# c-sommer/gradient-sdf

Measured on AMD Instinct MI355X. Metric: depth frames/sec fused+tracked, 640x480 @1cm voxels, higher is better.
Workload: dtype f32; 1 GPU; S-tum: TUM fr1/xyz-format synthetic stream, 640x480, 1 cm voxels, trunc 10, capacity 2^22 (BASELINE.json configs[1]); width=640, height=480, hash_capacity_log2=22, tracker=25 iters, conv 1e-3, damping 1, next_depth_hint=True, parallelism=replicas x1 (tracked path does not shard), full=False, burn_in_windows=2, converged_frames=20, voxels=1169329, n_upd_per_frame=4508803, n_hit_per_pass=254696

## Files before the change

gradient-sdf_amd/csrc/gsdf_capi.hip:

```cpp
#include "../../include/gsdf.h"
#include "../../include/gsdf_mc_tables.h"
#include "gsdf_ctx.h"
#include "gsdf_kernels.h"
#include "gsdf_math.h"

#include <hip/hip_runtime.h>

#include <algorithm>
#include <chrono>
#include <cmath>
#include <cstdio>
#include <cstdlib>
#include <cstring>
#include <numeric>
#include <string>
#include <thread>
#include <vector>

static int fail(int code, const std::string& msg) { return gsdf_fail(code, msg); }

namespace {

hipEvent_t take_event(gsdf_ctx* c) {
    if (!c->event_pool.empty()) {
        hipEvent_t e = c->event_pool.back();
        c->event_pool.pop_back();
        return e;
    }
    hipEvent_t e = nullptr;
    (void)hipEventCreateWithFlags(&e, hipEventDisableSystemFence);
    return e;
}

struct prof_scope {
    gsdf_ctx* c; int which; hipEvent_t a = nullptr, b = nullptr;
    prof_scope(gsdf_ctx* c_, int w) : c(c_), which(w) {
        if (c->profiling) { a = take_event(c); b = take_event(c); (void)hipEventRecord(a, c->stream); }
    }
    ~prof_scope() {
        if (c->profiling) { (void)hipEventRecord(b, c->stream); c->prof_events[which].push_back({ a, b }); }
    }
};

void prof_collect(gsdf_ctx* c) {
    for (int k = 0; k < GSDF_PROF_SLOTS; ++k) {
        for (auto& pr : c->prof_events[k]) {
            float ms = 0.f;
            if (hipEventElapsedTime(&ms, pr.first, pr.second) == hipSuccess) {
                c->prof_ms[k] += ms; c->prof_n[k] += 1;
                if (c->prof_each[k].size() < (size_t)1 << 20) c->prof_each[k].push_back(ms);
            }
            c->event_pool.push_back(pr.first);
            c->event_pool.push_back(pr.second);
        }
        c->prof_events[k].clear();
    }
}

int status_to_code(int status) {
    if (status & GSDF_STATUS_TABLE_FULL) return fail(GSDF_ERR_TABLE_FULL, "voxel hash table full (probe budget exhausted)");
    if (status & GSDF_STATUS_KEY_RANGE) return fail(GSDF_ERR_KEY_RANGE, "voxel index outside the packable +-2^20 range");
    if (status & GSDF_STATUS_TRACK_ABORT)
        return fail(GSDF_ERR_HIP, "tracking: the workgroups of the one-launch optimize() were not co-resident (GPU shared with another "
                                  "process?); that optimize() was abandoned -- set GSDF_PERSIST=0 to use one launch per pass");
    return GSDF_OK;
}

int require_frame(gsdf_ctx* c) {
    if (!c) return fail(GSDF_ERR_INVALID, "null context");
    if (!c->frame.planes) return fail(GSDF_ERR_INVALID, "gsdf_normals_init must be called first (NEst == nullptr, MapGradPixelSdf.cpp:55-58)");
    return GSDF_OK;
}

static int fuse_far_table(const gsdf_ctx* c) {
#ifdef GSDF_EXPERIMENTS
    if (c->debug & 1024) return 1;
    if (c->debug & 2048) return 0;
#endif
    if (c->far_table >= 0) return c->far_table;
    return c->progress && c->progress[3] * 16u > (unsigned int)c->fuse_blocks ? 1 : 0;
}

static inline void cpu_relax() {
#if defined(__x86_64__) || defined(__i386__)
    __builtin_ia32_pause();
#else
    std::this_thread::yield();
// ... 323 lines not shown
}

}

int gsdf_flush_pending(gsdf_ctx* c) {
    if (!c || !c->ahead.pending.valid) return GSDF_OK;
    c->ahead.release();
    if (hipSetDevice(c->device) != hipSuccess) return fail(GSDF_ERR_HIP, "hipSetDevice");
    const size_t N = (size_t)c->W * c->H;
    const gsdf_lookahead::pending_fuse& p = c->ahead.pending;
    return launch_fuse(c, p.depth, c->frame.normals + (size_t)p.set * 3 * N, p.pose, 0, fuse_far_table(c), nullptr, nullptr);
}
#define GSDF_FLUSH(c) do { if ((c) && (c)->ahead.pending.valid) { const int rc_ = gsdf_flush_pending(c); if (rc_) return rc_; } } while (0)
static int flush_if_overlaps(gsdf_ctx* c, const void* dst, int64_t bytes) {
    if (c && c->ahead.range_changes(dst, (size_t)std::max<int64_t>(bytes, 0), c->frame_bytes())) return gsdf_flush_pending(c);
    return GSDF_OK;
}

extern "C" {

const char* gsdf_last_error(void) { return g_gsdf_err.c_str(); }
#ifdef GSDF_EXPERIMENTS
#define GSDF_TRACE_WG 8192
#define GSDF_TRACE_COLS 16
int gsdf_debug_flags(gsdf_ctx* c, int flags) {
    GSDF_FLUSH(c);
    if (!c) return GSDF_ERR_INVALID;
    c->debug = flags;
    if (flags & 64) {
        if (hipStreamSynchronize(c->stream) != hipSuccess) return GSDF_ERR_HIP;
        if (!c->trace && c->trace.alloc((size_t)GSDF_TRACE_WG * GSDF_TRACE_COLS) != hipSuccess) return GSDF_ERR_HIP;
        if (hipMemset(c->trace, 0, (size_t)GSDF_TRACE_WG * GSDF_TRACE_COLS * 8) != hipSuccess) return GSDF_ERR_HIP;
        const unsigned long long ptr = (unsigned long long)(uintptr_t)c->trace.get();
        if (hipMemcpy(&c->st->dbg[23], &ptr, 8, hipMemcpyHostToDevice) != hipSuccess) return GSDF_ERR_HIP;
    }
    return GSDF_OK;
}
int gsdf_debug_trace(gsdf_ctx* c, unsigned long long* out, int n_wg) {
    GSDF_FLUSH(c);
    if (!c || !out || !c->trace || n_wg > GSDF_TRACE_WG) return GSDF_ERR_INVALID;
    if (hipStreamSynchronize(c->stream) != hipSuccess) return GSDF_ERR_HIP;
    if (hipMemcpy(out, c->trace, (size_t)n_wg * GSDF_TRACE_COLS * 8, hipMemcpyDeviceToHost) != hipSuccess) return GSDF_ERR_HIP;
    return GSDF_OK;
}
int gsdf_debug_raycast_rows(gsdf_ctx* c, unsigned long long* out, int n_rows) {
    GSDF_FLUSH(c);
    if (!c || !out || !c->rc_counts || (size_t)n_rows > c->rc_counts.count() / 8) return GSDF_ERR_INVALID;
    if (hipStreamSynchronize(c->stream) != hipSuccess) return GSDF_ERR_HIP;
    if (hipMemcpy(out, c->rc_counts, (size_t)n_rows * 8 * sizeof(unsigned long long), hipMemcpyDeviceToHost) != hipSuccess) return GSDF_ERR_HIP;
    return GSDF_OK;
}
int gsdf_debug_tile_counters(gsdf_ctx* c, unsigned long long* out, int n_rows) {
    GSDF_FLUSH(c);
    if (!c || !out || !c->frame.blk_counters || n_rows > c->fuse_blocks) return GSDF_ERR_INVALID;
    if (hipStreamSynchronize(c->stream) != hipSuccess) return GSDF_ERR_HIP;
    if (hipMemcpy(out, c->frame.blk_counters, (size_t)n_rows * 4 * sizeof(unsigned long long), hipMemcpyDeviceToHost) != hipSuccess) return GSDF_ERR_HIP;
    return GSDF_OK;
}
int gsdf_debug_set_tile_order(gsdf_ctx* c, const uint32_t* order, int n) {
    GSDF_FLUSH(c);
    if (!c || !order || !c->frame.tile_order || n != c->fuse_blocks) return GSDF_ERR_INVALID;
    if (hipStreamSynchronize(c->stream) != hipSuccess) return GSDF_ERR_HIP;
    if (hipMemcpy(c->frame.tile_order, order, (size_t)n * sizeof(uint32_t), hipMemcpyHostToDevice) != hipSuccess) return GSDF_ERR_HIP;
    return GSDF_OK;
}
int gsdf_debug_get_tile_order(gsdf_ctx* c, uint32_t* order, int* n) {
    if (!c || !order || !n || !c->frame.tile_order) return GSDF_ERR_INVALID;
    if (hipMemcpy(order, c->frame.tile_order, (size_t)c->fuse_blocks * sizeof(uint32_t), hipMemcpyDeviceToHost) != hipSuccess) return GSDF_ERR_HIP;
    *n = c->fuse_blocks;
    return GSDF_OK;
}
int gsdf_debug_read(gsdf_ctx* c, unsigned long long out[24]) {
    GSDF_FLUSH(c);
    if (!c || !out) return GSDF_ERR_INVALID;
    if (hipStreamSynchronize(c->stream) != hipSuccess) return GSDF_ERR_HIP;
    gsdf_dev_state h;
    if (hipMemcpy(&h, c->st, sizeof(h), hipMemcpyDeviceToHost) != hipSuccess) return GSDF_ERR_HIP;
    for (int i = 0; i < 24; ++i) out[i] = h.dbg[i];
    return GSDF_OK;
}
int gsdf_debug_normals_tile_split(int tiles, int k, int launches, int iters, int batch, int nrm_split, int nrm_split2, int* lo, int* hi) {
    return lo && hi && normals_tile_split(tiles, k, launches, iters, batch, nrm_split, nrm_split2, lo, hi) ? 1 : 0;
}
int gsdf_debug_fail_alloc(int nth) {
    const int made = g_gsdf_alloc_count;
    g_gsdf_alloc_count = 0;
    g_gsdf_alloc_fail_at = nth > 0 ? nth : 0;
    return made;
}
const char* gsdf_version(void) { return "gsdf-mi355x 0.2 (gfx950) +experiments"; }
#else
const char* gsdf_version(void) { return "gsdf-mi355x 0.2 (gfx950)"; }
#endif

static int create_impl(gsdf_ctx** out, float voxel_size, float trunc_dist, int capacity_log2, int device, bool other_queue);
int gsdf_create(gsdf_ctx** out, float voxel_size, float trunc_dist, int capacity_log2, int device) {
    return create_impl(out, voxel_size, trunc_dist, capacity_log2, device, false);
}
int gsdf_create_shards(gsdf_ctx** out, int n, float voxel_size, float trunc_dist, int capacity_log2, int device) {
    if (!out || n < 1 || n > 4) return fail(GSDF_ERR_INVALID, "gsdf_create_shards: 1..4 contexts (one hardware queue each)");
    for (int i = 0; i < n; ++i) out[i] = nullptr;
    for (int i = 0; i < n; ++i) {
        const int rc = create_impl(&out[i], voxel_size, trunc_dist, capacity_log2, device, true);
        if (rc) { for (int j = 0; j < i; ++j) { gsdf_destroy(out[j]); out[j] = nullptr; } return rc; }
    }
    return GSDF_OK;
}
static int create_impl(gsdf_ctx** out, float voxel_size, float trunc_dist, int capacity_log2, int device, bool other_queue) {
    if (!out) return fail(GSDF_ERR_INVALID, "out == NULL");
    *out = nullptr;
    if (!(voxel_size > 0.f) || !(trunc_dist > 0.f)) return fail(GSDF_ERR_INVALID, "voxel_size and trunc_dist must be > 0");
    if (capacity_log2 < 10 || capacity_log2 > 30) return fail(GSDF_ERR_INVALID, "capacity_log2 must be in [10, 30]");
    if (!(trunc_dist < 2.f)) return fail(GSDF_ERR_INVALID, "trunc_dist must be < 2 m (fixed-point range of the fusion kernel's accumulators)");
    int n_dev = 0;
    if (hipGetDeviceCount(&n_dev) != hipSuccess || n_dev <= 0) {
        (void)hipGetLastError();
        return fail(GSDF_ERR_NO_DEVICE, "no HIP device visible: libgsdf has no CPU fallback");
    }
    if (device < 0 || device >= n_dev) return fail(GSDF_ERR_INVALID, "device ordinal out of range");
    HIP_TRY(hipSetDevice(device));
    gsdf_ctx* c = new gsdf_ctx();
    c->device = device;
    c->voxel_size = voxel_size;
    c->voxel_size_inv = (float)(1. / voxel_size);
    c->T = trunc_dist;
    c->inv_T = (float)(1. / trunc_dist);
    c->factor = (int)std::floor(c->T / c->voxel_size);
    c->capacity_log2 = capacity_log2;
    c->n_slots = (size_t)1 << capacity_log2;
    hipError_t e;
    int prio_least = 0, prio_greatest = 0;
    if (other_queue) {
        if (hipDeviceGetStreamPriorityRange(&prio_least, &prio_greatest) != hipSuccess || prio_greatest == prio_least) {
            (void)hipGetLastError();
            delete c;
            return fail(GSDF_ERR_HIP, "gsdf_create_shards: the device offers no stream priority range, so separate hardware queues cannot be guaranteed (use gsdf_create)");
        }
    }
    if ((e = (other_queue ? hipStreamCreateWithPriority(&c->stream, hipStreamNonBlocking, prio_greatest)
                          : hipStreamCreateWithFlags(&c->stream, hipStreamNonBlocking))) != hipSuccess ||
        (e = c->map.alloc(c->n_slots, 0)) != hipSuccess || (e = c->st.alloc(1)) != hipSuccess || (e = c->counter.alloc(1)) != hipSuccess ||
        (e = hipEventCreate(&c->ev0)) != hipSuccess || (e = hipEventCreate(&c->ev1)) != hipSuccess) {
        std::string m = std::string("gsdf_create: ") + hipGetErrorString(e);
        gsdf_destroy(c);
        return fail(GSDF_ERR_HIP, m);
    }
    {
        const char* env = getenv("GSDF_DEFER");
        if (env) c->defer = atoi(env);
    }
    c->tab = c->map.table(c->n_slots);
    {
        if (c->progress.alloc(16) != hipSuccess) (void)hipGetLastError();
        const char* env = getenv("GSDF_ADAPTIVE");
        if (env) c->adaptive = atoi(env);
        if ((env = getenv("GSDF_FIRST_BATCH")) && atoi(env) >= 2) c->first_batch = atoi(env);
        if ((env = getenv("GSDF_FUSE_HEAD"))) c->fuse_head = atoi(env) != 0;
        if ((env = getenv("GSDF_NRM_SPLIT"))) {
            int a = -1, b = -1;
            const int n = sscanf(env, "%d,%d", &a, &b);
            if (n >= 1 && a >= 0 && a <= 100) { c->nrm_split = a; c->nrm_split2 = 100 - a; }
            if (n >= 2 && b >= 0 && a + b <= 100) c->nrm_split2 = b;
        }
        if ((env = getenv("GSDF_NEXT_BATCH")) && atoi(env) >= 1) c->next_batch = atoi(env);
        if ((env = getenv("GSDF_LAZY_FUSE"))) c->lazy_fuse = atoi(env);
        if ((env = getenv("GSDF_PERSIST"))) c->persist = atoi(env);
// ... 1098 lines not shown
```

gradient-sdf_amd/csrc/gsdf_kernels.hip:

```cpp
#include "gsdf_kernels.h"

#ifdef GSDF_EXPERIMENTS
#define GSDF_EXPERIMENT(flags, mask) (((flags) & (mask)) != 0)
#define GSDF_TRACE(a, tr, col) do { if (GSDF_EXPERIMENT((a).debug, 64) && threadIdx.x == 0) (tr)[col] = wall_clock64(); } while (0)
#else
#define GSDF_EXPERIMENT(flags, mask) (false)
#define GSDF_TRACE(a, tr, col) do { } while (0)
#endif
#include "gsdf_math.h"

#include <hip/hip_runtime.h>
#include <algorithm>
#include <cstring>
#include <vector>

#define FULL_MASK 0xFFFFFFFFFFFFFFFFull

template <int CTRL, int ROW_MASK>
__device__ __forceinline__ float dpp_add(float v) {
    const int moved = __builtin_amdgcn_update_dpp(0, __float_as_int(v), CTRL, ROW_MASK, 0xf, false);
    return v + __int_as_float(moved);
}
__device__ __forceinline__ float wave_sum(float v) {
    v = dpp_add<0x111, 0xf>(v);
    v = dpp_add<0x112, 0xf>(v);
    v = dpp_add<0x114, 0xf>(v);
    v = dpp_add<0x118, 0xf>(v);
    v = dpp_add<0x142, 0xa>(v);
    v = dpp_add<0x143, 0xc>(v);
    return __int_as_float(__builtin_amdgcn_readlane(__float_as_int(v), 63));
}

template <int CTRL, int ROW_MASK>
__device__ __forceinline__ uint32_t dpp_umin(uint32_t v) {
    const uint32_t m = (uint32_t)__builtin_amdgcn_update_dpp((int)0xFFFFFFFFu, (int)v, CTRL, ROW_MASK, 0xf, false);
    return m < v ? m : v;
}
template <int CTRL, int ROW_MASK>
__device__ __forceinline__ uint32_t dpp_umax(uint32_t v) {
    const uint32_t m = (uint32_t)__builtin_amdgcn_update_dpp(0, (int)v, CTRL, ROW_MASK, 0xf, false);
    return m > v ? m : v;
}
__device__ __forceinline__ void wave_uminmax(uint32_t& lo, uint32_t& hi) {
    lo = dpp_umin<0x111, 0xf>(lo); hi = dpp_umax<0x111, 0xf>(hi);
    lo = dpp_umin<0x112, 0xf>(lo); hi = dpp_umax<0x112, 0xf>(hi);
    lo = dpp_umin<0x114, 0xf>(lo); hi = dpp_umax<0x114, 0xf>(hi);
    lo = dpp_umin<0x118, 0xf>(lo); hi = dpp_umax<0x118, 0xf>(hi);
    lo = dpp_umin<0x142, 0xa>(lo); hi = dpp_umax<0x142, 0xa>(hi);
    lo = dpp_umin<0x143, 0xc>(lo); hi = dpp_umax<0x143, 0xc>(hi);
    lo = (uint32_t)__builtin_amdgcn_readlane((int)lo, 63);
    hi = (uint32_t)__builtin_amdgcn_readlane((int)hi, 63);
}

#define GSDF_DPP_STAGE(CTRL)                                                                     \
    _Pragma("unroll") for (int i = 0; i < N; ++i)                                                \
        asm volatile("v_add_f32_dpp %0, %0, %0 " CTRL : "+v"(v[i]))
template <int N>
__device__ __forceinline__ void wave_sum_to_lane63(float (&v)[N]) {
    static_assert(N >= 3, "DPP read-after-write distance");
    if constexpr (N == 29) {
        asm volatile("s_nop 1" : "+v"(v[0]), "+v"(v[1]), "+v"(v[2]), "+v"(v[3]), "+v"(v[4]), "+v"(v[5]), "+v"(v[6]), "+v"(v[7]), "+v"(v[8]),
                     "+v"(v[9]), "+v"(v[10]), "+v"(v[11]), "+v"(v[12]), "+v"(v[13]), "+v"(v[14]), "+v"(v[15]), "+v"(v[16]), "+v"(v[17]), "+v"(v[18]),
                     "+v"(v[19]), "+v"(v[20]), "+v"(v[21]), "+v"(v[22]), "+v"(v[23]), "+v"(v[24]), "+v"(v[25]), "+v"(v[26]), "+v"(v[27]), "+v"(v[28]));
    } else {
#pragma unroll
        for (int i = 0; i < N; ++i) asm volatile("s_nop 1" : "+v"(v[i]));
    }
    GSDF_DPP_STAGE("row_shr:1 row_mask:0xf bank_mask:0xf bound_ctrl:1");
    GSDF_DPP_STAGE("row_shr:2 row_mask:0xf bank_mask:0xf bound_ctrl:1");
    GSDF_DPP_STAGE("row_shr:4 row_mask:0xf bank_mask:0xf bound_ctrl:1");
    GSDF_DPP_STAGE("row_shr:8 row_mask:0xf bank_mask:0xf bound_ctrl:1");
    GSDF_DPP_STAGE("row_bcast:15 row_mask:0xa bank_mask:0xf");
    GSDF_DPP_STAGE("row_bcast:31 row_mask:0xc bank_mask:0xf");
}
#undef GSDF_DPP_STAGE

__device__ __forceinline__ int reflect101(int i, int n) {
    if (n == 1) return 0;
    while (i < 0 || i >= n) {
        if (i < 0) i = -i;
        else i = 2 * (n - 1) - i;
    }
    return i;
}

__global__ __launch_bounds__(256) void k_table_clear(gsdf_table tab, size_t n_blocks) {
    const size_t stride = (size_t)gridDim.x * blockDim.x;
    const size_t n16 = n_blocks * GSDF_BLOCK_VOX * 2;
    uint4* p = reinterpret_cast<uint4*>(tab.vox);
    for (size_t i = (size_t)blockIdx.x * blockDim.x + threadIdx.x; i < n16; i += stride) p[i] = make_uint4(0u, 0u, 0u, 0u);
    for (size_t i = (size_t)blockIdx.x * blockDim.x + threadIdx.x; i < n_blocks; i += stride) tab.bkeys[i] = GSDF_KEY_EMPTY;
    const size_t n_occ = ((size_t)gsdf_occ_mask(tab) + 1) / 32 + ((size_t)gsdf_occ2_mask(tab) + 1) / 32;
// ... 1279 lines not shown
    float trig[4] = { 0.f, 1.f, 0.f, 1.f };
    const float theta_sq = gsdf_se3_theta_sq(xi);
    if (!(theta_sq < GSDF_SOPHUS_EPS * GSDF_SOPHUS_EPS)) {
        const float theta = sqrtf(theta_sq), half = 0.5f * theta;
        const float arg = (threadIdx.x & 1u) ? theta : half;
        const float sn = sinf(arg), cs = cosf(arg);
        trig[0] = trk_lane_value(sn, 0); trig[1] = trk_lane_value(cs, 0);
        trig[2] = trk_lane_value(sn, 1); trig[3] = trk_lane_value(cs, 1);
    }
    gsdf_se3_exp_mul_trig(xi, pose7, trig);
}
__device__ __forceinline__ float trk_sin_small(float x, float x2) {
    float p = __builtin_fmaf(x2, -1.f / 5040.f, 1.f / 120.f);
    p = __builtin_fmaf(x2, p, -1.f / 6.f);
    return __builtin_fmaf(x, x2 * p, x);
}
__device__ __forceinline__ float trk_cos_small(float x2) {
    float p = __builtin_fmaf(x2, -1.f / 720.f, 1.f / 24.f);
    p = __builtin_fmaf(x2, p, -0.5f);
    return __builtin_fmaf(x2, p, 1.f);
}
__device__ __forceinline__ void trk_se3_exp_mul_fast(const float* xi, float* pose7) {
    const float theta_sq = gsdf_se3_theta_sq(xi);
    if (__builtin_expect(!(theta_sq >= GSDF_SOPHUS_EPS * GSDF_SOPHUS_EPS && theta_sq < 0.01f), 0)) {
        trk_se3_exp_mul_wave(xi, pose7);
        return;
    }
    const float rth = trk_rsq(theta_sq);
    const float theta = theta_sq * rth, half = 0.5f * theta;
    const float tsq = theta * theta, hsq = half * half;
    const float rth2 = rth * rth;
    const float imag = trk_sin_small(half, hsq) * rth;
    const float real = trk_cos_small(hsq);
    const float a = (1.f - trk_cos_small(tsq)) * rth2;
    const float b = (theta - trk_sin_small(theta, tsq)) * (rth2 * rth);
    float qn[4];
    gsdf_se3_exp_mul_parts(xi, pose7, imag, real, false, a, b, qn);
    const float rl = trk_rsq(qn[0] * qn[0] + qn[1] * qn[1] + qn[2] * qn[2] + qn[3] * qn[3]);
#pragma unroll
    for (int i = 0; i < 4; ++i) pose7[3 + i] = qn[i] * rl;
}

__device__ __forceinline__ void trk_solve_update(const float* tot, float damping, float conv_sq, int passes, int max_passes,
                                                 int no_solve, bool exact_solve ,
                                                 float pose[7], int* done, int* converged) {
    float gvec[6], Hm[36];
#pragma unroll
    for (int i = 0; i < 6; ++i) gvec[i] = tot[1 + i];
    int q = 7;
#pragma unroll
    for (int i = 0; i < 6; ++i)
#pragma unroll
        for (int j = i; j < 6; ++j) { Hm[6 * i + j] = tot[q]; Hm[6 * j + i] = tot[q]; ++q; }
    float xi[6];
    if (no_solve) { for (int i = 0; i < 6; ++i) xi[i] = 1.f; }
    else if (exact_solve || __builtin_expect(!trk_llt_solve6_fast(Hm, gvec, xi), 0))
        gsdf_llt_solve6(Hm, gvec, xi);
#pragma unroll
    for (int i = 0; i < 6; ++i) xi[i] = damping * xi[i];
    const float nrm = gsdf_sum3(xi[0] * xi[0], xi[1] * xi[1], xi[2] * xi[2]) +
                      gsdf_sum3(xi[3] * xi[3], xi[4] * xi[4], xi[5] * xi[5]);
    *done = 0; *converged = 0;
    if (nrm < conv_sq) {
        *converged = 1;
        *done = 1;
    } else {
        bool nan = false;
#pragma unroll
        for (int i = 0; i < 6; ++i) nan = nan || isnan(xi[i]);
        if (!nan && !no_solve) {
            float mxi[6];
#pragma unroll
            for (int i = 0; i < 6; ++i) mxi[i] = -xi[i];
            if (exact_solve) trk_se3_exp_mul_wave(mxi, pose);
            else trk_se3_exp_mul_fast(mxi, pose);
        }
        if (passes >= max_passes) *done = 1;
    }
}

template <int PPT>
__device__ __forceinline__ void trk_gather(const gsdf_frame_geom& g, const gsdf_table& tab, const float* __restrict__ depth,
                                           const float* z_first, const float pose[7], int pix0, int pix_stride, int batch_stride,
                                           float (&acc)[GSDF_TRACK_NSUM], unsigned long long* wave_stamp = nullptr,
                                           const int xy_scale = 1) {
    const unsigned long long ws_t0 = wave_stamp ? wall_clock64() : 0ull;
    float R[9];
    gsdf_quat_to_R(pose + 3, R);
    const float t[3] = { pose[0], pose[1], pose[2] };
    const float fx_inv = 1.f / g.fx, fy_inv = 1.f / g.fy;
    const int N = g.W * g.H;
    const uint32_t uW = (uint32_t)g.W;
    const uint32_t step_y = (uint32_t)pix_stride / uW, step_x = (uint32_t)pix_stride - step_y * uW;
    for (int base = pix0; base < N; base += batch_stride) {
        float z[PPT];
        bool ok[PPT];
#pragma unroll
        for (int j = 0; j < PPT; ++j) {
            const int pix = base + j * pix_stride;
            ok[j] = pix < N;
            z[j] = (z_first && base == pix0) ? z_first[j] : (ok[j] ? depth[pix] : 0.f);
        }
        gsdf_v3 p[PPT];
        int vx[PPT], vy[PPT], vz[PPT];
        unsigned long long key[PPT], bkey[PPT], k0[PPT];
        uint32_t home[PPT];
        uint32_t px, py = (uint32_t)base / uW;
        px = (uint32_t)base - py * uW;
#pragma unroll
        for (int j = 0; j < PPT; ++j) {
            ok[j] = ok[j] && !(z[j] <= g.zmin || z[j] >= g.zmax);
            const int y = (int)py * xy_scale, x = (int)px * xy_scale;
            px += step_x; py += step_y;
            if (px >= uW) { px -= uW; ++py; }
            const float x0 = ((float)x - g.cx) * fx_inv;
            const float y0 = ((float)y - g.cy) * fy_inv;
            const gsdf_v3 pc = { x0 * z[j], y0 * z[j], z[j] };
            const gsdf_v3 Rp = gsdf_matvec(R, pc);
            p[j] = gsdf_v3{ Rp.x + t[0], Rp.y + t[1], Rp.z + t[2] };
            vx[j] = gsdf_float2vox1(g.inv_vs, p[j].x);
            vy[j] = gsdf_float2vox1(g.inv_vs, p[j].y);
            vz[j] = gsdf_float2vox1(g.inv_vs, p[j].z);
            ok[j] = ok[j] && gsdf_key_in_range(vx[j], vy[j], vz[j]);
            key[j] = gsdf_key_pack(vx[j], vy[j], vz[j]);
            bkey[j] = gsdf_block_key(key[j]);
            home[j] = gsdf_hash(bkey[j]) & tab.block_mask;
            k0[j] = ok[j] ? tab.bkeys[home[j]] : GSDF_KEY_EMPTY;
        }
        const gsdf_payload* P[PPT];
        float2 pa[PPT], pb[PPT], pc2[PPT];
        int blk[PPT];
        {
            uint32_t want = 0u;
#pragma unroll
            for (int j = 0; j < PPT; ++j) want |= ok[j] ? 1u << j : 0u;
            gsdf_block_lookup_n<PPT, false>(tab, bkey, home, k0, want, blk);
        }
        unsigned long long ws_lookup = 0ull, ws_ok = 0ull;
        if (wave_stamp && base == pix0) {
            ws_lookup = wall_clock64() - ws_t0;
#pragma unroll
            for (int j = 0; j < PPT; ++j) ws_ok += (unsigned long long)__popcll(__ballot(ok[j]));
        }
#pragma unroll
        for (int j = 0; j < PPT; ++j) {
            P[j] = blk[j] >= 0 ? tab.vox + ((size_t)blk[j] * GSDF_BLOCK_VOX + gsdf_block_local(key[j])) : nullptr;
            if (P[j]) {
                const float2* q = reinterpret_cast<const float2*>(P[j]);
                pa[j] = q[0]; pb[j] = q[1]; pc2[j] = q[2];
            } else {
                pa[j] = make_float2(0.f, 0.f); pb[j] = pa[j]; pc2[j] = pa[j];
            }
        }
#pragma unroll
        for (int j = 0; j < PPT; ++j) {
            const float w0 = pa[j].x;
            if (!(w0 > 0.f)) continue;
            const gsdf_v3 gn = gsdf_normalized3(gsdf_v3{ pb[j].x, pb[j].y, pc2[j].x });
            const gsdf_v3 gr = { 1.2f * gn.x, 1.2f * gn.y, 1.2f * gn.z };
            const gsdf_v3 d = { g.vs * (float)vx[j] - p[j].x, g.vs * (float)vy[j] - p[j].y, g.vs * (float)vz[j] - p[j].z };
            const float phi = gsdf_tsdf_phi(pa[j].y / w0, gn, d);
            const gsdf_v3 pxg = gsdf_cross3(p[j], gr);
            const float J[6] = { gr.x, gr.y, gr.z, pxg.x, pxg.y, pxg.z };
            acc[0] += phi * phi;
#pragma unroll
            for (int i = 0; i < 6; ++i) acc[1 + i] += phi * J[i];
            int q = 7;
#pragma unroll
            for (int i = 0; i < 6; ++i)
#pragma unroll
                for (int jj = i; jj < 6; ++jj) acc[q++] += J[i] * J[jj];
            acc[28] += 1.f;
        }
        if (wave_stamp && base == pix0) {
            unsigned long long hits = 0ull;
#pragma unroll
            for (int j = 0; j < PPT; ++j) hits += (unsigned long long)__popcll(__ballot(pa[j].x > 0.f));
            const unsigned long long tot = wall_clock64() - ws_t0;
            if ((threadIdx.x & 63) == 0)
                *wave_stamp = (tot & 0xFFFFull) | ((ws_lookup & 0xFFFFull) << 16) | ((ws_ok & 0xFFFFull) << 32) | ((hits & 0xFFFFull) << 48);
        }
    }
}

struct base_sample {
    float w;
    float phi;
    gsdf_v3 grad;
};
__device__ __forceinline__ base_sample gsdf_base_sample(const gsdf_table& tab, float inv_vs, float T, gsdf_v3 p) {
    const float pi = inv_vs * p.x, pj = inv_vs * p.y, pk = inv_vs * p.z;
    const int im = (int)floorf(pi), jm = (int)floorf(pj), km = (int)floorf(pk);
    const float dx = pi - (float)im, dy = pj - (float)jm, dz = pk - (float)km;
    const uint32_t inx = (gsdf_key_in_range(im, 0, 0) ? 1u : 0u) | (gsdf_key_in_range(im + 1, 0, 0) ? 2u : 0u);
    const uint32_t iny = (gsdf_key_in_range(0, jm, 0) ? 1u : 0u) | (gsdf_key_in_range(0, jm + 1, 0) ? 2u : 0u);
    const uint32_t inz = (gsdf_key_in_range(0, 0, km) ? 1u : 0u) | (gsdf_key_in_range(0, 0, km + 1) ? 2u : 0u);
    const uint32_t span = ((im & 3) == 3 ? 1u : 0u) | ((jm & 3) == 3 ? 2u : 0u) | ((km & 3) == 3 ? 4u : 0u);
    unsigned long long bk[8], k[8];
    uint32_t h[8];
    int blk[8];
    uint32_t pend = 0u;
#pragma unroll
    for (int e = 0; e < 8; ++e) {
        const int i0 = e & 1, j0 = (e >> 1) & 1, k0 = (e >> 2) & 1;
        const bool want = (e & ~span) == 0u && ((inx >> i0) & 1u) && ((iny >> j0) & 1u) && ((inz >> k0) & 1u);
        bk[e] = want ? gsdf_block_key(gsdf_key_pack(im + i0, jm + j0, km + k0)) : 0ull;
        h[e] = gsdf_hash(bk[e]) & tab.block_mask;
        k[e] = want ? tab.bkeys[h[e]] : GSDF_KEY_EMPTY;
        pend |= want ? 1u << e : 0u;
    }
    gsdf_block_lookup_n<8, false>(tab, bk, h, k, pend, blk);
    float d[8], wv[8];
    uint32_t present = 0u;
#pragma unroll
    for (int c = 0; c < 8; ++c) {
        int b = blk[0];
#pragma unroll
        for (int e = 1; e < 8; ++e)
            if ((e & ~c) == 0) b = (uint32_t)e == (c & span) ? blk[e] : b;
// ... 28 lines not shown
    const float d13 = (1.f - dy) * d[1] + dy * d[3];
    const float d46 = (1.f - dy) * d[4] + dy * d[6];
    const float d57 = (1.f - dy) * d[5] + dy * d[7];
    r.grad.x = inv_vs * ((1.f - dz) * d13 + dz * d57 - (1.f - dz) * d02 - dz * d46);
    r.grad.y = inv_vs * ((1.f - dz) * d23 + dz * d67 - (1.f - dz) * d01 - dz * d45);
    r.grad.z = inv_vs * ((1.f - dy) * d45 + dy * d67 - (1.f - dy) * d01 - dy * d23);
    const float dy0 = (1.f - dy) * d01 + dy * d23;
    const float dy1 = (1.f - dy) * d45 + dy * d67;
    r.phi = (1.f - dz) * dy0 + dz * dy1;
    return r;
}

template <int PPT>
__device__ __forceinline__ void trk_gather_base(const gsdf_frame_geom& g, const gsdf_table& tab, const float* __restrict__ depth,
                                                const float pose[7], int pix0, int pix_stride, int batch_stride,
                                                float (&acc)[GSDF_TRACK_NSUM], const int xy_scale = 1) {
    float R[9];
    gsdf_quat_to_R(pose + 3, R);
    const float t[3] = { pose[0], pose[1], pose[2] };
    const float fx_inv = 1.f / g.fx, fy_inv = 1.f / g.fy;
    const int N = g.W * g.H;
    const uint32_t uW = (uint32_t)g.W;
#pragma unroll 1
    for (int base = pix0; base < N; base += batch_stride) {
#pragma unroll 1
        for (int j = 0; j < PPT; ++j) {
            const int pix = base + j * pix_stride;
            if (pix >= N) break;
            const float z = depth[pix];
            if (z <= g.zmin || z >= g.zmax) continue;
            const uint32_t py = (uint32_t)pix / uW, px = (uint32_t)pix - py * uW;
            const int y = (int)py * xy_scale, x = (int)px * xy_scale;
            const float x0 = ((float)x - g.cx) * fx_inv;
            const float y0 = ((float)y - g.cy) * fy_inv;
            const gsdf_v3 pc = { x0 * z, y0 * z, z };
            const gsdf_v3 Rp = gsdf_matvec(R, pc);
            const gsdf_v3 p = { Rp.x + t[0], Rp.y + t[1], Rp.z + t[2] };
            const base_sample bs = gsdf_base_sample(tab, g.inv_vs, g.T, p);
            if (!(bs.w > 0.f)) continue;
            const float phi = bs.phi;
            const gsdf_v3 gr = bs.grad;
            const gsdf_v3 pxg = gsdf_cross3(p, gr);
            const float J[6] = { gr.x, gr.y, gr.z, pxg.x, pxg.y, pxg.z };
            acc[0] += phi * phi;
#pragma unroll
            for (int i = 0; i < 6; ++i) acc[1 + i] += phi * J[i];
            int q = 7;
#pragma unroll
            for (int i = 0; i < 6; ++i)
#pragma unroll
                for (int jj = i; jj < 6; ++jj) acc[q++] += J[i] * J[jj];
            acc[28] += 1.f;
        }
    }
}

static_assert(GSDF_TRACK_BLOCK == NRM_THREADS, "the normals tiles of the first pass run in tracker-sized workgroups");
template <bool SAMPLED, bool BASE>
__global__ __launch_bounds__(GSDF_TRACK_BLOCK, BASE ? 2 : 4) void k_track_pass(gsdf_frame_geom g, const float* __restrict__ depth,
                                                                            gsdf_table tab, gsdf_dev_state* st,
                                                                            double* rows, gsdf_track_params tp, gsdf_normals_job nj) {
    if ((int)blockIdx.x >= tp.n_track_blocks) {
        extern __shared__ __attribute__((aligned(16))) unsigned char dyn_lds[];
        if (nj.token && st->nrm_token == nj.token) return;
        const int t = (int)blockIdx.x - tp.n_track_blocks + nj.tile_first;
        if (t == 0 && threadIdx.x == 0) {
            *nj.deferred_count = 0u;
            st->frame_cur = st->frames;
        }
        normals_tile(*reinterpret_cast<nrm_lds*>(dyn_lds), t % nj.ntx, t / nj.ntx, g.W, g.H, nj.r, nj.nc, depth, nj.nx, nj.ny, nj.nz,
                     gsdf_tile_stats{ nj.stats, (g.W + 15) / 16, g.zmin, g.zmax });
        return;
    }
    unsigned long long* trk_tr = nullptr;
    if (GSDF_EXPERIMENT(tp.debug, 64) && blockIdx.x < 512u && tp.pass_index < 12) {
        trk_tr = reinterpret_cast<unsigned long long*>(st->dbg[23]) + 16 * (2048 + (size_t)tp.pass_index * 512 + blockIdx.x);
        if (threadIdx.x == 0) trk_tr[0] = wall_clock64();
    }
    __shared__ float wsum[GSDF_TRACK_BLOCK / 64][32];
    __shared__ float sh_pose[8];
    __shared__ int sh_done;
    const int tid = threadIdx.x, lane = tid & 63, wave = tid >> 6;
    const int k = tp.pass_index;
    float pose[7];
    const bool trk_heavy = wave < GSDF_TRACK_BLOCK / 128;
    const int trk_pix0 = (int)blockIdx.x * TRK_CHUNK + (trk_heavy ? wave * (64 * TRK_PPT) : (GSDF_TRACK_BLOCK / 128) * 64 * TRK_PPT + (wave - GSDF_TRACK_BLOCK / 128) * (64 * (TRK_PPT - 1))) + lane;
    const int trk_batch = tp.n_track_blocks * TRK_CHUNK;
    float z_pre[TRK_PPT];
    {
        const int N = g.W * g.H;
#pragma unroll
        for (int j = 0; j < TRK_PPT; ++j) {
            const int pix = trk_pix0 + j * 64;
            z_pre[j] = (pix < N && (trk_heavy || j < TRK_PPT - 1)) ? depth[pix] : 0.f;
        }
    }
    double* acc_cur = rows + (size_t)(tp.rot % 3u) * GSDF_TRACK_ROWSET;
    const double* acc_prev = rows + (size_t)((tp.rot + 2u) % 3u) * GSDF_TRACK_ROWSET;
    if (blockIdx.x == 0) {
        double* nxt = rows + (size_t)((tp.rot + 1u) % 3u) * GSDF_TRACK_ROWSET;
        for (int i = threadIdx.x; i < GSDF_TRACK_ROWSET; i += GSDF_TRACK_BLOCK) nxt[i] = 0.0;
    }

    if (k > 0 && tp.head_done) {
        const gsdf_trk_buf& cur = st->trk[k & 1];
        if (cur.done) return;
#pragma unroll
        for (int i = 0; i < 7; ++i) pose[i] = cur.pose7[i];
    } else if (k == 0) {
#pragma unroll
        for (int i = 0; i < 7; ++i) pose[i] = st->pose7[i];
        if (blockIdx.x == 0 && tid == 0) {
            gsdf_trk_buf& o = st->trk[0];
#pragma unroll
            for (int i = 0; i < 7; ++i) o.pose7[i] = pose[i];
            o.done = 0; o.converged = 0; o.passes = 0;
            st->done = 0; st->converged = 0;
        }
    } else {
        const gsdf_trk_buf& in = st->trk[(k - 1) & 1];
        if (GSDF_EXPERIMENT(tp.debug, 8) && wave != 0) {
            float pose_old[7];
#pragma unroll
            for (int i = 0; i < 7; ++i) pose_old[i] = in.pose7[i];
            float dummy[GSDF_TRACK_NSUM];
#pragma unroll
            for (int i = 0; i < GSDF_TRACK_NSUM; ++i) dummy[i] = 0.f;
            const int xy_scale_w = SAMPLED ? tp.sampling : 1;
            if constexpr (BASE) {
                if (trk_heavy) trk_gather_base<TRK_PPT>(g, tab, depth, pose_old, trk_pix0, 64, trk_batch, dummy, xy_scale_w);
                else trk_gather_base<TRK_PPT - 1>(g, tab, depth, pose_old, trk_pix0, 64, trk_batch, dummy, xy_scale_w);
            } else {
                if (trk_heavy) trk_gather<TRK_PPT>(g, tab, depth, z_pre, pose_old, trk_pix0, 64, trk_batch, dummy, nullptr, xy_scale_w);
                else trk_gather<TRK_PPT - 1>(g, tab, depth, z_pre, pose_old, trk_pix0, 64, trk_batch, dummy, nullptr, xy_scale_w);
            }
            if (dummy[28] == -1.f) st->dbg[20] = 1ull;
        }
        if (wave == 0) {
            double gs = 0.0;
            if (lane < GSDF_TRACK_NSUM) {
                double part[GSDF_TRACK_GROUPS];
#pragma unroll
                for (int grp = 0; grp < GSDF_TRACK_GROUPS; ++grp) part[grp] = acc_prev[grp * 32 + lane];
                gs = part[0];
#pragma unroll
                for (int grp = 1; grp < GSDF_TRACK_GROUPS; ++grp) gs += part[grp];
            }
            const int in_done = in.done;
#pragma unroll
            for (int i = 0; i < 7; ++i) pose[i] = in.pose7[i];
            const int passes = in.passes + 1;
            if (trk_tr && threadIdx.x == 0) { trk_tr[4] = wall_clock64() + (unsigned long long)(gs != gs) + (unsigned long long)(passes < 0); }
            int done = 1, converged = 0;
            if (!in_done) {
                const float totv = (float)gs;
                float tot[GSDF_TRACK_NSUM];
#pragma unroll
                for (int i = 0; i < GSDF_TRACK_NSUM; ++i) tot[i] = __int_as_float(__builtin_amdgcn_readlane(__float_as_int(totv), i));
                trk_solve_update(tot, tp.damping, tp.conv_sq, passes, tp.max_passes, GSDF_EXPERIMENT(tp.debug, 1), GSDF_EXPERIMENT(tp.debug, 4), pose, &done, &converged);
                if (trk_tr && threadIdx.x == 0) trk_tr[5] = wall_clock64() + (unsigned long long)(pose[0] != pose[0]);
                if (blockIdx.x == 0 && tid == 0) {
                    gsdf_trk_buf& o = st->trk[k & 1];
#pragma unroll
                    for (int i = 0; i < 7; ++i) { o.pose7[i] = pose[i]; st->pose7[i] = pose[i]; }
                    o.done = done; o.converged = converged; o.passes = passes;
                    if (done) st->trk[(k - 1) & 1].done = 1;
                    gsdf_quat_to_R(pose + 3, st->R);
                    st->converged = converged;
                    st->done = done;
                    st->passes = passes;
                    st->last_hits = tot[28];
                    st->n_hit += (unsigned long long)tot[28];
                    if (tp.progress)
                        __hip_atomic_store(&tp.progress[0], (tp.serial << 16) | (done ? 0x8000u : 0u) | (unsigned int)(passes & 0x7FFF),
                                           __ATOMIC_RELAXED, __HIP_MEMORY_SCOPE_SYSTEM);
                }
            }
            if (lane == 0) {
#pragma unroll
                for (int i = 0; i < 7; ++i) sh_pose[i] = pose[i];
                sh_done = done;
            }
        }
        __syncthreads();
        if (sh_done) return;
#pragma unroll
        for (int i = 0; i < 7; ++i) pose[i] = sh_pose[i];
    }
    if (trk_tr && threadIdx.x == 0) trk_tr[1] = wall_clock64();
    if (k >= tp.max_passes || GSDF_EXPERIMENT(tp.debug, 2)) return;

    float acc[GSDF_TRACK_NSUM];
#pragma unroll
    for (int i = 0; i < GSDF_TRACK_NSUM; ++i) acc[i] = 0.f;
    const int xy_scale = SAMPLED ? tp.sampling : 1;
    if constexpr (BASE) {
        if (trk_heavy) trk_gather_base<TRK_PPT>(g, tab, depth, pose, trk_pix0, 64, trk_batch, acc, xy_scale);
        else trk_gather_base<TRK_PPT - 1>(g, tab, depth, pose, trk_pix0, 64, trk_batch, acc, xy_scale);
    } else {
        if (trk_heavy) trk_gather<TRK_PPT>(g, tab, depth, z_pre, pose, trk_pix0, 64, trk_batch, acc, trk_tr ? trk_tr + 8 + wave : nullptr, xy_scale);
        else trk_gather<TRK_PPT - 1>(g, tab, depth, z_pre, pose, trk_pix0, 64, trk_batch, acc, trk_tr ? trk_tr + 8 + wave : nullptr, xy_scale);
    }
    if (trk_tr && threadIdx.x == 0) trk_tr[2] = wall_clock64();
    wave_sum_to_lane63(acc);
    if (lane == 63) {
#pragma unroll
        for (int i = 0; i < GSDF_TRACK_NSUM; ++i) wsum[wave][i] = acc[i];
    }
    if (trk_tr && threadIdx.x == 0) trk_tr[6] = wall_clock64();
    __syncthreads();
    if (trk_tr && threadIdx.x == 0) trk_tr[7] = wall_clock64();
    if (tid < 32) {
        float v = 0.f;
        if (tid < GSDF_TRACK_NSUM) {
            v = wsum[0][tid];
#pragma unroll
            for (int w = 1; w < GSDF_TRACK_BLOCK / 64; ++w) v += wsum[w][tid];
        }
        if (tid < GSDF_TRACK_NSUM) unsafeAtomicAdd(&acc_cur[(blockIdx.x % GSDF_TRACK_GROUPS) * 32 + tid], (double)v);
    }
    if (trk_tr && threadIdx.x == 0) trk_tr[3] = wall_clock64();
}
int gsdf_normals_tiles(int W, int H) { return ((W + NRM_TX - 1) / NRM_TX) * ((H + NRM_TY - 1) / NRM_TY); }
void gsdf_launch_track_pass(hipStream_t s, const gsdf_frame_geom& g, const float* depth, gsdf_table tab,
                            gsdf_dev_state* st, double* partials, int n_blocks, const gsdf_track_params& tp_in,
                            const gsdf_normals_job* normals, int base) {
    gsdf_track_params tp = tp_in;
    {
        const int chunks = std::max(1, (g.W * g.H + TRK_CHUNK - 1) / TRK_CHUNK), cap = std::max(1, n_blocks);
        const int per = (chunks + cap - 1) / cap;
        n_blocks = (chunks + per - 1) / per;
    }
    if (tp.pass_index >= tp.max_passes && !normals) n_blocks = 1;
    tp.n_track_blocks = n_blocks;
    gsdf_normals_job nj;
    memset(&nj, 0, sizeof(nj));
    int extra = 0;
    size_t dyn = 0;
    if (normals) {
        nj = *normals;
        nj.ntx = (g.W + NRM_TX - 1) / NRM_TX;
        const int rest = nj.ntx * ((g.H + NRM_TY - 1) / NRM_TY) - nj.tile_first;
        extra = std::max(0, nj.tile_count > 0 ? std::min(nj.tile_count, rest) : rest);
        dyn = extra ? sizeof(nrm_lds) : 0;
    }
    if (base) {
        if (tp.sampling > 1)
            hipLaunchKernelGGL((k_track_pass<true, true>), dim3(n_blocks + extra), dim3(GSDF_TRACK_BLOCK), dyn, s, g, depth, tab, st, partials, tp, nj);
        else
            hipLaunchKernelGGL((k_track_pass<false, true>), dim3(n_blocks + extra), dim3(GSDF_TRACK_BLOCK), dyn, s, g, depth, tab, st, partials, tp, nj);
    } else if (tp.sampling > 1)
        hipLaunchKernelGGL((k_track_pass<true, false>), dim3(n_blocks + extra), dim3(GSDF_TRACK_BLOCK), dyn, s, g, depth, tab, st, partials, tp, nj);
    else
        hipLaunchKernelGGL((k_track_pass<false, false>), dim3(n_blocks + extra), dim3(GSDF_TRACK_BLOCK), dyn, s, g, depth, tab, st, partials, tp, nj);
}

__global__ __launch_bounds__(256) void k_subsample(const float* __restrict__ depth, int W, int s, int Ws, int Ns, float* __restrict__ out) {
    const int q = (int)(blockIdx.x * blockDim.x + threadIdx.x);
    if (q >= Ns) return;
    const int qy = q / Ws, qx = q - qy * Ws;
    out[q] = depth[(size_t)(qy * s) * W + (size_t)qx * s];
}
void gsdf_launch_subsample(hipStream_t st, const float* depth, int W, int H, int s, float* out) {
    const int Ws = (W + s - 1) / s, Hs = (H + s - 1) / s, Ns = Ws * Hs;
    hipLaunchKernelGGL(k_subsample, dim3((Ns + 255) / 256), dim3(256), 0, st, depth, W, s, Ws, Ns, out);
}

#define TRK_ROW_CHUNKS 10
__device__ __forceinline__ gsdf_u32x4 trk_load_chunk(const gsdf_u32x4* p) {
    gsdf_u32x4 v;
    asm volatile("global_load_dwordx4 %0, %1, off sc1" : "=v"(v) : "v"(p) : "memory");
    return v;
}
template <int MAXB>
__global__ __launch_bounds__(GSDF_TRACK_BLOCK) void k_track_all(gsdf_frame_geom g, const float* __restrict__ depth, gsdf_table tab,
                                                                gsdf_dev_state* st, gsdf_u32x4* rows ,
                                                                unsigned int* abort_word, gsdf_track_params tp, gsdf_normals_job nj) {
    if ((int)blockIdx.x >= tp.n_track_blocks) {
        extern __shared__ __attribute__((aligned(16))) unsigned char dyn_lds[];
        const int t = (int)blockIdx.x - tp.n_track_blocks;
        if (t == 0 && threadIdx.x == 0) {
            *nj.deferred_count = 0u;
            st->frame_cur = st->frames;
        }
        normals_tile(*reinterpret_cast<nrm_lds*>(dyn_lds), t % nj.ntx, t / nj.ntx, g.W, g.H, nj.r, nj.nc, depth, nj.nx, nj.ny, nj.nz,
                     gsdf_tile_stats{ nj.stats, (g.W + 15) / 16, g.zmin, g.zmax });
        return;
    }
    constexpr int NW = GSDF_TRACK_BLOCK / 64;
    __shared__ float wsum[NW][32];
    __shared__ double part[16][32];
    extern __shared__ __attribute__((aligned(16))) unsigned char dyn_lds_t[];
    float (*rowv)[3 * TRK_ROW_CHUNKS] = reinterpret_cast<float (*)[3 * TRK_ROW_CHUNKS]>(dyn_lds_t);
    const int tid = threadIdx.x, lane = tid & 63, wave = tid >> 6;
    const int nb = tp.n_track_blocks;
    const int n_chunks = nb * TRK_ROW_CHUNKS;
    unsigned long long* trk_tr = nullptr;
    if (GSDF_EXPERIMENT(tp.debug, 64) && blockIdx.x < 512u)
        trk_tr = reinterpret_cast<unsigned long long*>(st->dbg[23]) + 16 * (2048 + (size_t)blockIdx.x);
    float z_pre[TRK_PPT];
    {
        const int N = g.W * g.H, base0 = (int)blockIdx.x * GSDF_TRACK_BLOCK + tid, nthreads = nb * GSDF_TRACK_BLOCK;
#pragma unroll
        for (int j = 0; j < TRK_PPT; ++j) {
            const int pix = base0 + j * nthreads;
            z_pre[j] = pix < N ? depth[pix] : 0.f;
        }
    }
    float pose[7];
#pragma unroll
    for (int i = 0; i < 7; ++i) pose[i] = st->pose7[i];
    int done = 0, converged = 0, passes = 0;
    float hits = 0.f;
    unsigned long long hit_total = 0ull;
    bool aborted = false;
    for (int k = 0; k < tp.max_passes && !done; ++k) {
        if (trk_tr && tid == 0 && k < 12) trk_tr[16 * 512 * k + 0] = wall_clock64();
        float acc[GSDF_TRACK_NSUM];
#pragma unroll
        for (int i = 0; i < GSDF_TRACK_NSUM; ++i) acc[i] = 0.f;
        trk_gather<TRK_PPT>(g, tab, depth, z_pre, pose, blockIdx.x * GSDF_TRACK_BLOCK + tid, nb * GSDF_TRACK_BLOCK, TRK_PPT * nb * GSDF_TRACK_BLOCK, acc);
        if (trk_tr && tid == 0 && k < 12) trk_tr[16 * 512 * k + 1] = wall_clock64();
        wave_sum_to_lane63(acc);
        if (lane == 63) {
#pragma unroll
            for (int i = 0; i < GSDF_TRACK_NSUM; ++i) wsum[wave][i] = acc[i];
        }
        __syncthreads();
        const uint32_t tag = (tp.serial << 8) | (uint32_t)(k + 1);
        gsdf_u32x4* buf = rows + (size_t)(k & 1) * (size_t)n_chunks;
        if (tid < TRK_ROW_CHUNKS) {
            float v3[3];
#pragma unroll
            for (int q = 0; q < 3; ++q) {
                const int i = 3 * tid + q;
                float v = 0.f;
                if (i < GSDF_TRACK_NSUM) {
                    v = wsum[0][i];
#pragma unroll
                    for (int w = 1; w < NW; ++w) v += wsum[w][i];
                }
                v3[q] = v;
            }
            const gsdf_u32x4 c = { __float_as_uint(v3[0]), __float_as_uint(v3[1]), __float_as_uint(v3[2]), tag };
            gsdf_u32x4* dst = buf + (size_t)blockIdx.x * TRK_ROW_CHUNKS + tid;
            asm volatile("global_store_dwordx4 %0, %1, off sc1" :: "v"(dst), "v"(c) : "memory");
        }
        if (trk_tr && tid == 0 && k < 12) trk_tr[16 * 512 * k + 2] = wall_clock64();
        constexpr int PER = (MAXB * TRK_ROW_CHUNKS + GSDF_TRACK_BLOCK - 1) / GSDF_TRACK_BLOCK;
        gsdf_u32x4 ch[PER];
        const unsigned long long t0 = wall_clock64();
        unsigned int rounds = 0u;
        for (;;) {
            bool ok = true;
#pragma unroll
            for (int i = 0; i < PER; ++i) {
                const int c = tid + GSDF_TRACK_BLOCK * i;
                ch[i] = gsdf_u32x4{ 0u, 0u, 0u, tag };
                if (c < n_chunks) ch[i] = trk_load_chunk(buf + c);
            }
#pragma unroll
            for (int i = 0; i < PER; ++i) asm volatile("s_waitcnt vmcnt(0)" : "+v"(ch[i]) :: "memory");
#pragma unroll
            for (int i = 0; i < PER; ++i) ok = ok && ch[i].w == tag;
            ++rounds;
            if (__syncthreads_and(ok ? 1 : 0)) break;
            if (__hip_atomic_load(abort_word, __ATOMIC_RELAXED, __HIP_MEMORY_SCOPE_AGENT) == tp.serial || wall_clock64() - t0 > 5000000ull) {
                aborted = true;
                break;
            }
            __builtin_amdgcn_s_sleep(2);
        }
        if (aborted) {
            if (tid == 0) {
                __hip_atomic_store(abort_word, tp.serial, __ATOMIC_RELAXED, __HIP_MEMORY_SCOPE_AGENT);
                atomicOr(&st->status, GSDF_STATUS_TRACK_ABORT);
            }
            break;
        }
        if (trk_tr && tid == 0 && k < 12) { trk_tr[16 * 512 * k + 3] = wall_clock64(); trk_tr[16 * 512 * k + 6] = rounds; }
#pragma unroll
        for (int i = 0; i < PER; ++i) {
            const int c = tid + GSDF_TRACK_BLOCK * i;
            if (c < n_chunks) {
                const int r = c / TRK_ROW_CHUNKS, q = c - r * TRK_ROW_CHUNKS;
                rowv[r][3 * q] = __uint_as_float(ch[i].x); rowv[r][3 * q + 1] = __uint_as_float(ch[i].y); rowv[r][3 * q + 2] = __uint_as_float(ch[i].z);
            }
        }
        __syncthreads();
        {
            const int v = tid & 31, grp = tid >> 5;
            const int per = (nb + 15) / 16;
            double sgrp = 0.0;
            if (v < 3 * TRK_ROW_CHUNKS)
                for (int r = grp * per; r < (grp + 1) * per && r < nb; ++r) sgrp += (double)rowv[r][v];
            part[grp][v] = sgrp;
        }
        __syncthreads();
        float tot[GSDF_TRACK_NSUM];
        {
            double gs = 0.0;
            if (lane < GSDF_TRACK_NSUM) {
                gs = part[0][lane];
#pragma unroll
// ... 608 lines not shown
```

Baseline: 10370 frames/s.

## Deduplicate hash block lookups per wave via run-length compaction of block keys

```diff
diff --git a/gradient-sdf_amd/csrc/gsdf_capi.hip b/gradient-sdf_amd/csrc/gsdf_capi.hip
--- a/gradient-sdf_amd/csrc/gsdf_capi.hip
+++ b/gradient-sdf_amd/csrc/gsdf_capi.hip
@@ -3,6 +3,7 @@
 #include "gsdf_ctx.h"
 #include "gsdf_kernels.h"
 #include "gsdf_math.h"
+#include "gsdf_runs.h"
 
 #include <hip/hip_runtime.h>
 
@@ -492,6 +493,27 @@
 int gsdf_debug_normals_tile_split(int tiles, int k, int launches, int iters, int batch, int nrm_split, int nrm_split2, int* lo, int* hi) {
     return lo && hi && normals_tile_split(tiles, k, launches, iters, batch, nrm_split, nrm_split2, lo, hi) ? 1 : 0;
 }
+int gsdf_debug_track_rows(gsdf_ctx* c, double* out) {
+    GSDF_FLUSH(c);
+    if (!c || !out || !c->frame.partials) return GSDF_ERR_INVALID;
+    if (hipStreamSynchronize(c->stream) != hipSuccess) return GSDF_ERR_HIP;
+    if (hipMemcpy(out, c->frame.partials, (size_t)3 * GSDF_TRACK_ROWSET * sizeof(double), hipMemcpyDeviceToHost) != hipSuccess) return GSDF_ERR_HIP;
+    return GSDF_OK;
+}
+int gsdf_debug_run_plan(const unsigned long long* valid, const unsigned long long* differs, int rows, int* pos,
+                        unsigned long long* leaders, int* count, int* rounds) {
+    if (!valid || !differs || !pos || !leaders || !count || !rounds || rows < 0) return 0;
+    int n = 0;
+    for (int j = 0; j < rows; ++j) {
+        const uint64_t lead = gsdf_run_leaders(valid[j], differs[j]);
+        for (int l = 0; l < GSDF_RUN_LANES; ++l) pos[j * GSDF_RUN_LANES + l] = ((valid[j] >> l) & 1ull) ? gsdf_run_pos(lead, n, l) : -1;
+        leaders[j] = lead;
+        n += gsdf_run_popcount(lead);
+    }
+    *count = n;
+    *rounds = gsdf_run_rounds(n);
+    return 1;
+}
 int gsdf_debug_fail_alloc(int nth) {
     const int made = g_gsdf_alloc_count;
     g_gsdf_alloc_count = 0;
diff --git a/gradient-sdf_amd/csrc/gsdf_kernels.hip b/gradient-sdf_amd/csrc/gsdf_kernels.hip
--- a/gradient-sdf_amd/csrc/gsdf_kernels.hip
+++ b/gradient-sdf_amd/csrc/gsdf_kernels.hip
@@ -8,6 +8,7 @@
 #define GSDF_TRACE(a, tr, col) do { } while (0)
 #endif
 #include "gsdf_math.h"
+#include "gsdf_runs.h"
 
 #include <hip/hip_runtime.h>
 #include <algorithm>
@@ -1453,8 +1454,9 @@
 template <int PPT>
 __device__ __forceinline__ void trk_gather(const gsdf_frame_geom& g, const gsdf_table& tab, const float* __restrict__ depth,
                                            const float* z_first, const float pose[7], int pix0, int pix_stride, int batch_stride,
-                                           float (&acc)[GSDF_TRACK_NSUM], unsigned long long* wave_stamp = nullptr,
-                                           const int xy_scale = 1) {
+                                           float (&acc)[GSDF_TRACK_NSUM], unsigned long long* runs,
+                                           unsigned long long* wave_stamp = nullptr, const int xy_scale = 1,
+                                           const bool per_pixel = false, unsigned long long* multi_round = nullptr) {
     const unsigned long long ws_t0 = wave_stamp ? wall_clock64() : 0ull;
     float R[9];
     gsdf_quat_to_R(pose + 3, R);
@@ -1463,7 +1465,7 @@
     const int N = g.W * g.H;
     const uint32_t uW = (uint32_t)g.W;
     const uint32_t step_y = (uint32_t)pix_stride / uW, step_x = (uint32_t)pix_stride - step_y * uW;
-    for (int base = pix0; base < N; base += batch_stride) {
+    for (int base = pix0; __builtin_amdgcn_readfirstlane(base) < N; base += batch_stride) {
         float z[PPT];
         bool ok[PPT];
 #pragma unroll
@@ -1474,8 +1476,7 @@
         }
         gsdf_v3 p[PPT];
         int vx[PPT], vy[PPT], vz[PPT];
-        unsigned long long key[PPT], bkey[PPT], k0[PPT];
-        uint32_t home[PPT];
+        unsigned long long key[PPT], bkey[PPT];
         uint32_t px, py = (uint32_t)base / uW;
         px = (uint32_t)base - py * uW;
 #pragma unroll
@@ -1495,17 +1496,57 @@
             ok[j] = ok[j] && gsdf_key_in_range(vx[j], vy[j], vz[j]);
             key[j] = gsdf_key_pack(vx[j], vy[j], vz[j]);
             bkey[j] = gsdf_block_key(key[j]);
-            home[j] = gsdf_hash(bkey[j]) & tab.block_mask;
-            k0[j] = ok[j] ? tab.bkeys[home[j]] : GSDF_KEY_EMPTY;
         }
         const gsdf_payload* P[PPT];
         float2 pa[PPT], pb[PPT], pc2[PPT];
         int blk[PPT];
-        {
+        if (per_pixel) {
+            unsigned long long k0[PPT];
+            uint32_t home[PPT];
             uint32_t want = 0u;
 #pragma unroll
-            for (int j = 0; j < PPT; ++j) want |= ok[j] ? 1u << j : 0u;
+            for (int j = 0; j < PPT; ++j) {
+                home[j] = gsdf_hash(bkey[j]) & tab.block_mask;
+                k0[j] = ok[j] ? tab.bkeys[home[j]] : GSDF_KEY_EMPTY;
+                want |= ok[j] ? 1u << j : 0u;
+            }
             gsdf_block_lookup_n<PPT, false>(tab, bkey, home, k0, want, blk);
+        } else {
+            int* const runs_i = reinterpret_cast<int*>(runs);
+            int pos[PPT];
+            int count = 0;
+#pragma unroll
+            for (int j = 0; j < PPT; ++j) {
+                const int lo = (int)(uint32_t)bkey[j], hi = (int)(uint32_t)(bkey[j] >> 32);
+                const int plo = __builtin_amdgcn_update_dpp(lo, lo, 0x138, 0xF, 0xF, false);
+                const int phi = __builtin_amdgcn_update_dpp(hi, hi, 0x138, 0xF, 0xF, false);
+                const uint64_t lead = gsdf_run_leaders(__ballot(ok[j]), __ballot(plo != lo || phi != hi));
+                const uint64_t below = gsdf_run_pos_mask(lead);
+                pos[j] = gsdf_run_pos_base(lead, count) +
+                         (int)__builtin_amdgcn_mbcnt_hi((uint32_t)(below >> 32), __builtin_amdgcn_mbcnt_lo((uint32_t)below, 0u));
+                if (__builtin_amdgcn_inverse_ballot_w64(lead)) runs[pos[j]] = bkey[j];
+                count += gsdf_run_popcount(lead);
+            }
+            __builtin_amdgcn_fence(__ATOMIC_ACQ_REL, "wavefront");
+            __builtin_amdgcn_wave_barrier();
+            const int lane = (int)__lane_id();
+            for (int first = 0; first < count; first += GSDF_RUN_LANES) {
+                const int i = first + lane;
+                const bool mine = i < count;
+                const unsigned long long bk1[1] = { mine ? runs[i] : 0ull };
+                uint32_t h1[1] = { gsdf_hash(bk1[0]) & tab.block_mask };
+                unsigned long long k1[1] = { mine ? tab.bkeys[h1[0]] : GSDF_KEY_EMPTY };
+                int b1[1];
+                gsdf_block_lookup_n<1, false>(tab, bk1, h1, k1, mine ? 1u : 0u, b1);
+                if (mine) runs_i[2 * i] = b1[0];
+            }
+            if (multi_round && count > GSDF_RUN_LANES && lane == 0) atomicAdd(multi_round, 1ull);
+            __builtin_amdgcn_fence(__ATOMIC_ACQ_REL, "wavefront");
+            __builtin_amdgcn_wave_barrier();
+#pragma unroll
+            for (int j = 0; j < PPT; ++j) blk[j] = ok[j] ? runs_i[2 * pos[j]] : -1;
+            __builtin_amdgcn_fence(__ATOMIC_ACQ_REL, "wavefront");
+            __builtin_amdgcn_wave_barrier();
         }
         unsigned long long ws_lookup = 0ull, ws_ok = 0ull;
         if (wave_stamp && base == pix0) {
@@ -1700,6 +1741,12 @@
     __shared__ int sh_done;
     const int tid = threadIdx.x, lane = tid & 63, wave = tid >> 6;
     const int k = tp.pass_index;
+    unsigned long long* trk_runs = nullptr;
+    if constexpr (!BASE) {
+        __shared__ unsigned long long sh_runs[GSDF_TRACK_BLOCK / 64][TRK_PPT * GSDF_RUN_LANES];
+        trk_runs = sh_runs[wave];
+    }
+    const bool trk_per_pixel = GSDF_EXPERIMENT(tp.debug, 16);
     float pose[7];
     const bool trk_heavy = wave < GSDF_TRACK_BLOCK / 128;
     const int trk_pix0 = (int)blockIdx.x * TRK_CHUNK + (trk_heavy ? wave * (64 * TRK_PPT) : (GSDF_TRACK_BLOCK / 128) * 64 * TRK_PPT + (wave - GSDF_TRACK_BLOCK / 128) * (64 * (TRK_PPT - 1))) + lane;
@@ -1749,8 +1796,8 @@
                 if (trk_heavy) trk_gather_base<TRK_PPT>(g, tab, depth, pose_old, trk_pix0, 64, trk_batch, dummy, xy_scale_w);
                 else trk_gather_base<TRK_PPT - 1>(g, tab, depth, pose_old, trk_pix0, 64, trk_batch, dummy, xy_scale_w);
             } else {
-                if (trk_heavy) trk_gather<TRK_PPT>(g, tab, depth, z_pre, pose_old, trk_pix0, 64, trk_batch, dummy, nullptr, xy_scale_w);
-                else trk_gather<TRK_PPT - 1>(g, tab, depth, z_pre, pose_old, trk_pix0, 64, trk_batch, dummy, nullptr, xy_scale_w);
+                if (trk_heavy) trk_gather<TRK_PPT>(g, tab, depth, z_pre, pose_old, trk_pix0, 64, trk_batch, dummy, trk_runs, nullptr, xy_scale_w, trk_per_pixel);
+                else trk_gather<TRK_PPT - 1>(g, tab, depth, z_pre, pose_old, trk_pix0, 64, trk_batch, dummy, trk_runs, nullptr, xy_scale_w, trk_per_pixel);
             }
             if (dummy[28] == -1.f) st->dbg[20] = 1ull;
         }
@@ -1816,8 +1863,9 @@
         if (trk_heavy) trk_gather_base<TRK_PPT>(g, tab, depth, pose, trk_pix0, 64, trk_batch, acc, xy_scale);
         else trk_gather_base<TRK_PPT - 1>(g, tab, depth, pose, trk_pix0, 64, trk_batch, acc, xy_scale);
     } else {
-        if (trk_heavy) trk_gather<TRK_PPT>(g, tab, depth, z_pre, pose, trk_pix0, 64, trk_batch, acc, trk_tr ? trk_tr + 8 + wave : nullptr, xy_scale);
-        else trk_gather<TRK_PPT - 1>(g, tab, depth, z_pre, pose, trk_pix0, 64, trk_batch, acc, trk_tr ? trk_tr + 8 + wave : nullptr, xy_scale);
+        unsigned long long* const trk_multi = GSDF_EXPERIMENT(1, 1) ? &st->dbg[21] : nullptr;
+        if (trk_heavy) trk_gather<TRK_PPT>(g, tab, depth, z_pre, pose, trk_pix0, 64, trk_batch, acc, trk_runs, trk_tr ? trk_tr + 8 + wave : nullptr, xy_scale, trk_per_pixel, trk_multi);
+        else trk_gather<TRK_PPT - 1>(g, tab, depth, z_pre, pose, trk_pix0, 64, trk_batch, acc, trk_runs, trk_tr ? trk_tr + 8 + wave : nullptr, xy_scale, trk_per_pixel, trk_multi);
     }
     if (trk_tr && threadIdx.x == 0) trk_tr[2] = wall_clock64();
     wave_sum_to_lane63(acc);
@@ -1908,6 +1956,7 @@
     constexpr int NW = GSDF_TRACK_BLOCK / 64;
     __shared__ float wsum[NW][32];
     __shared__ double part[16][32];
+    __shared__ unsigned long long sh_runs[NW][TRK_PPT * GSDF_RUN_LANES];
     extern __shared__ __attribute__((aligned(16))) unsigned char dyn_lds_t[];
     float (*rowv)[3 * TRK_ROW_CHUNKS] = reinterpret_cast<float (*)[3 * TRK_ROW_CHUNKS]>(dyn_lds_t);
     const int tid = threadIdx.x, lane = tid & 63, wave = tid >> 6;
@@ -1937,7 +1986,8 @@
         float acc[GSDF_TRACK_NSUM];
 #pragma unroll
         for (int i = 0; i < GSDF_TRACK_NSUM; ++i) acc[i] = 0.f;
-        trk_gather<TRK_PPT>(g, tab, depth, z_pre, pose, blockIdx.x * GSDF_TRACK_BLOCK + tid, nb * GSDF_TRACK_BLOCK, TRK_PPT * nb * GSDF_TRACK_BLOCK, acc);
+        trk_gather<TRK_PPT>(g, tab, depth, z_pre, pose, blockIdx.x * GSDF_TRACK_BLOCK + tid, nb * GSDF_TRACK_BLOCK, TRK_PPT * nb * GSDF_TRACK_BLOCK, acc,
+                            sh_runs[wave], nullptr, 1, GSDF_EXPERIMENT(tp.debug, 16), GSDF_EXPERIMENT(1, 1) ? &st->dbg[21] : nullptr);
         if (trk_tr && tid == 0 && k < 12) trk_tr[16 * 512 * k + 1] = wall_clock64();
         wave_sum_to_lane63(acc);
         if (lane == 63) {
diff --git a/gradient-sdf_amd/csrc/gsdf_runs.h b/gradient-sdf_amd/csrc/gsdf_runs.h
--- /dev/null
+++ b/gradient-sdf_amd/csrc/gsdf_runs.h
@@ -0,0 +1,25 @@
+#ifndef GSDF_RUNS_H_
+#define GSDF_RUNS_H_
+
+#include <stdint.h>
+
+#if defined(__HIPCC__)
+#define GSDF_RUNS_FN __host__ __device__ __forceinline__
+#else
+#define GSDF_RUNS_FN static inline
+#endif
+
+#define GSDF_RUN_LANES 64
+
+GSDF_RUNS_FN uint64_t gsdf_run_leaders(uint64_t valid, uint64_t differs) {
+    return valid & (differs | ~(valid << 1) | 1ull);
+}
+GSDF_RUNS_FN int gsdf_run_popcount(uint64_t m) { return __builtin_popcountll(m); }
+GSDF_RUNS_FN int gsdf_run_pos_base(uint64_t leaders, int row_off) { return row_off + (int)(leaders & 1ull) - 1; }
+GSDF_RUNS_FN uint64_t gsdf_run_pos_mask(uint64_t leaders) { return leaders >> 1; }
+GSDF_RUNS_FN int gsdf_run_pos(uint64_t leaders, int row_off, int lane) {
+    return gsdf_run_pos_base(leaders, row_off) + gsdf_run_popcount(gsdf_run_pos_mask(leaders) & ((1ull << lane) - 1ull));
+}
+GSDF_RUNS_FN int gsdf_run_rounds(int count) { return (count + GSDF_RUN_LANES - 1) / GSDF_RUN_LANES; }
+
+#endif
```

Measured after the change: 10390 frames/s, median of 5. Within noise of the previous version (+0.2%).
